# FintanH/rust-crdt

Hardware: AMD Instinct MI355X
Metric: replica-merges/sec (whole node) + achieved HBM GB/s as % of MI355X peak (higher is better)
Workload: dtype u64

## Files before the change

rust-crdt_amd/csrc/common.hpp:

```cpp
#pragma once

#include <hip/hip_runtime.h>

#include <cstdint>
#include <cstdio>
#include <algorithm>
#include <cstring>
#include <map>
#include <string>
#include <vector>

#include "crdt_gpu.h"
#include "shard_host.hpp"

namespace crdt {

using u64 = unsigned long long;
using u64x2 = unsigned long long __attribute__((ext_vector_type(2)));

constexpr int kWave = 64;

#ifndef CRDT_APPLY_WPE
#define CRDT_APPLY_WPE 0
#endif
// ... 62 lines not shown
  int wire_walk = 1;
  int wire_fill = 1;
  int host_stream = 1;
  int apply_lane = 1;
  int apply_fence = 0;
  int orswot_apply_pf = 0;
  int orswot_apply_stg = 0;
  int orswot_apply_l2pf = 0;
  int orswot_apply_meta = 1;
  int orswot_apply_hpf = 0;
  int map_counter_dma = 0;
  int map_counter_depth = 8;
  int map_counter_kpw = 0;
  int map_counter_cs = 1;
  int map_counter_cl = 0;
  int map_orswot_cs = 0;
  int map_orswot_wide = 0;
  int map_nested_lds = 1;
  int map_apply_meta = 1;
  int map_apply_pf = 1;
  int read_bpc = 0;
  int read_unroll = 8;
  int read_nt = 1;
  int eqv_ppl = 8;
  int eqv_bpc = 32;
  int rx_lds = 1;
};

struct PendingTiming {
  std::string name;
  hipEvent_t start, stop;
};

}

struct crdt_ctx {
  int device = 0;
  hipStream_t stream = nullptr;
  int cu_count = 256;
  bool timing = false;
  crdt::Tune tune;
  std::string last_error;
  void *scratch = nullptr;
  size_t scratch_bytes = 0;
  void *dscratch = nullptr;
  size_t dscratch_bytes = 0;
  unsigned *counters = nullptr;
  size_t counters_n = 0;
  void *pinned = nullptr;
  size_t pinned_bytes = 0;
  hipEvent_t pinned_done = nullptr;
  std::map<std::string, crdt::KernelTimer> timers;
  std::vector<crdt::PendingTiming> pending;
  std::vector<hipEvent_t> free_events;
  void *comm = nullptr;
  int nranks = 1, rank = 0;
  void (*comm_destroy)(void *) = nullptr;
  void *sbuf[8] = {};
  size_t sbuf_bytes[8] = {};
  bool has_ops = false;
  crdt_comm_ops ops{};
  hipStream_t astream = nullptr;
  hipEvent_t a_main = nullptr, a_done = nullptr;
  void *a_dev = nullptr, *a_host = nullptr;
  size_t a_rows = 0;
  std::string comm_note;
  void (*comm_release)(crdt_ctx *) = nullptr;
  crdt::shard_host::PlanCache plans;
  bool chk_pending = false;
  uint64_t chk_key = 0;
  void *chk_dev = nullptr;
  uint64_t *chk_host = nullptr;
  hipEvent_t chk_ev = nullptr;
  int (*comm_check)(crdt_ctx *) = nullptr;
  int mem_kind = CRDT_MEM_DEVICE;
  hipStream_t hstream = nullptr;
  void *hbuf[2] = {};
  size_t hbuf_bytes = 0;
  void *hacc = nullptr;
  size_t hacc_bytes = 0;
  hipEvent_t hcopied[2] = {}, hfree[2] = {};
};

namespace crdt {

int fail(crdt_ctx *ctx, int code, const char *fmt, ...);
int hip_fail(crdt_ctx *ctx, hipError_t e, const char *what);
int ensure_scratch(crdt_ctx *ctx, size_t bytes);
int ensure_dscratch(crdt_ctx *ctx, size_t bytes);
int ensure_counters(crdt_ctx *ctx, size_t n);
int stage_h2d(crdt_ctx *ctx, void *dst, const void *src, size_t bytes);
int device_fill(crdt_ctx *ctx, void *dst, size_t bytes, unsigned char byte);
void timing_begin(crdt_ctx *ctx, const char *name);
void timing_end(crdt_ctx *ctx);
void timing_add_host(crdt_ctx *ctx, const char *name, double ms);

struct DefPlan {
  const size_t *def_off;
  unsigned long long G, D, M, A, Mw;
  const u64 *def_clock, *def_members;
  const u64 *out_clock;
  u64 *out_entries;
  int apply_ceiling;
  u64 *hash;
  unsigned *surv;
  unsigned *nsurv;
  uint8_t *out_keep;
  u64 *out_members;
  u64 *tkey;
  unsigned *trep;
  unsigned long long tmask;
};
int launch_deferred(crdt_ctx *ctx, const size_t *host_def_off, DefPlan q, const u64 *dev_def_off = nullptr,
                    unsigned *status = nullptr);
int stage_def_off_dev(crdt_ctx *ctx, const u64 *src, size_t *dst, size_t G, size_t D, unsigned *status,
                      unsigned *flags);

enum class Op : int { Max = 0, Or = 1 };

template <Op OP>
__device__ __forceinline__ u64 join(u64 a, u64 b) {
  if constexpr (OP == Op::Max) return a > b ? a : b;
  else return a | b;
}
template <Op OP>
__device__ __forceinline__ u64x2 join2(u64x2 a, u64x2 b) {
  u64x2 r;
  r.x = join<OP>(a.x, b.x);
  r.y = join<OP>(a.y, b.y);
  return r;
}

int lattice_lub_many(crdt_ctx *ctx, Op op, const u64 *in, size_t G, size_t R, size_t W,
                     size_t row_stride, size_t group_stride, u64 *out, size_t out_stride,
                     unsigned flags);
int lattice_merge_batch(crdt_ctx *ctx, Op op, u64 *self, const u64 *other, size_t N, size_t W,
                        size_t self_stride, size_t other_stride);
struct LubReq {
  Op op;
  const u64 *in;
  size_t G, R, W, row_stride, group_stride;
  u64 *out;
  size_t out_stride;
  unsigned flags;
};
// ... 79 lines not shown
```

rust-crdt_amd/csrc/ctx.cpp:

```cpp
#include <cstdarg>
#include <cstdlib>

#include "common.hpp"

namespace crdt {

static thread_local std::string g_orphan_error;

int fail(crdt_ctx *ctx, int code, const char *fmt, ...) {
  char buf[512];
  va_list ap;
  va_start(ap, fmt);
  vsnprintf(buf, sizeof buf, fmt, ap);
  va_end(ap);
  if (ctx) ctx->last_error = buf;
  else g_orphan_error = buf;
  return code;
}

int hip_fail(crdt_ctx *ctx, hipError_t e, const char *what) {
  return fail(ctx, CRDT_EHIP, "%s failed: %s (%d)", what, hipGetErrorString(e), (int)e);
}

int ensure_scratch(crdt_ctx *ctx, size_t bytes) {
  if (bytes <= ctx->scratch_bytes) return CRDT_OK;
  if (ctx->scratch) {
    (void)hipStreamSynchronize(ctx->stream);
    (void)hipFree(ctx->scratch);
    ctx->scratch = nullptr;
    ctx->scratch_bytes = 0;
  }
  size_t want = bytes < (1u << 20) ? (1u << 20) : bytes + bytes / 4;
// ... 12 lines not shown
    (void)hipStreamSynchronize(ctx->stream);
    (void)hipFree(ctx->dscratch);
    ctx->dscratch = nullptr;
    ctx->dscratch_bytes = 0;
  }
  size_t want = bytes < (1u << 16) ? (1u << 16) : bytes + bytes / 4;
  hipError_t e = hipMalloc(&ctx->dscratch, want);
  if (e != hipSuccess) {
    ctx->dscratch = nullptr;
    return fail(ctx, CRDT_ENOMEM, "dscratch hipMalloc(%zu) failed: %s", want, hipGetErrorString(e));
  }
  ctx->dscratch_bytes = want;
  return CRDT_OK;
}

int ensure_counters(crdt_ctx *ctx, size_t n) {
  if (n <= ctx->counters_n) return CRDT_OK;
  if (ctx->counters) {
    (void)hipStreamSynchronize(ctx->stream);
    (void)hipFree(ctx->counters);
    ctx->counters = nullptr;
    ctx->counters_n = 0;
  }
  size_t want = n < 16384 ? 16384 : n * 2;
  hipError_t e = hipMalloc(&ctx->counters, want * sizeof(unsigned));
  if (e != hipSuccess) {
    ctx->counters = nullptr;
    return fail(ctx, CRDT_ENOMEM, "counter hipMalloc failed: %s", hipGetErrorString(e));
  }
  ctx->counters_n = want;
  return device_fill(ctx, ctx->counters, want * sizeof(unsigned), 0);
}

int stage_h2d(crdt_ctx *ctx, void *dst, const void *src, size_t bytes) {
  if (bytes == 0) return CRDT_OK;
  if (ctx->pinned_done) {
    hipError_t e = hipEventSynchronize(ctx->pinned_done);
    if (e != hipSuccess) return hip_fail(ctx, e, "hipEventSynchronize(pinned)");
  } else {
    hipError_t e = hipEventCreateWithFlags(&ctx->pinned_done, hipEventDisableTiming);
    if (e != hipSuccess) return hip_fail(ctx, e, "hipEventCreate(pinned)");
  }
  if (bytes > ctx->pinned_bytes) {
    if (ctx->pinned) (void)hipHostFree(ctx->pinned);
    ctx->pinned = nullptr;
    ctx->pinned_bytes = 0;
    size_t want = bytes < 65536 ? 65536 : bytes * 2;
    hipError_t e = hipHostMalloc(&ctx->pinned, want, hipHostMallocDefault);
    if (e != hipSuccess) return fail(ctx, CRDT_ENOMEM, "hipHostMalloc(%zu) failed", want);
    ctx->pinned_bytes = want;
  }
  std::memcpy(ctx->pinned, src, bytes);
  hipError_t e = hipMemcpyAsync(dst, ctx->pinned, bytes, hipMemcpyHostToDevice, ctx->stream);
  if (e != hipSuccess) return hip_fail(ctx, e, "hipMemcpyAsync(staged)");
  e = hipEventRecord(ctx->pinned_done, ctx->stream);
  if (e != hipSuccess) return hip_fail(ctx, e, "hipEventRecord(pinned)");
  return CRDT_OK;
}

__global__ void fill_u64_kernel(unsigned long long *p, size_t n, unsigned long long v) {
  for (size_t i = (size_t)blockIdx.x * blockDim.x + threadIdx.x; i < n; i += (size_t)gridDim.x * blockDim.x)
    p[i] = v;
}
__global__ void fill_u8_kernel(unsigned char *p, size_t n, unsigned char v) {
  for (size_t i = (size_t)blockIdx.x * blockDim.x + threadIdx.x; i < n; i += (size_t)gridDim.x * blockDim.x)
    p[i] = v;
}

int device_fill(crdt_ctx *ctx, void *dst, size_t bytes, unsigned char byte) {
  if (bytes == 0) return CRDT_OK;
  const bool wide = (reinterpret_cast<uintptr_t>(dst) % 8 == 0) && bytes % 8 == 0;
  const size_t n = wide ? bytes / 8 : bytes;
  size_t blocks = (n + kBlock - 1) / kBlock;
  const size_t cap = (size_t)ctx->cu_count * 8;
  if (blocks > cap) blocks = cap;
  if (wide)
    hipLaunchKernelGGL(fill_u64_kernel, dim3((unsigned)blocks), dim3(kBlock), 0, ctx->stream,
                       (unsigned long long *)dst, n, 0x0101010101010101ULL * byte);
  else
    hipLaunchKernelGGL(fill_u8_kernel, dim3((unsigned)blocks), dim3(kBlock), 0, ctx->stream,
                       (unsigned char *)dst, n, byte);
  hipError_t e = hipGetLastError();
  return e == hipSuccess ? CRDT_OK : hip_fail(ctx, e, "device_fill");
}

static hipEvent_t take_event(crdt_ctx *ctx) {
  if (!ctx->free_events.empty()) {
    hipEvent_t e = ctx->free_events.back();
    ctx->free_events.pop_back();
    return e;
// ... 135 lines not shown
int crdt_ctx_create(int device, crdt_ctx **out) {
  if (!out) return fail(nullptr, CRDT_EINVAL, "crdt_ctx_create: out is NULL");
  *out = nullptr;
  int n = 0;
  hipError_t e = hipGetDeviceCount(&n);
  if (e != hipSuccess || n == 0)
    return fail(nullptr, CRDT_EHIP, "crdt_ctx_create: no HIP device (%s)", hipGetErrorString(e));
  if (device < 0 || device >= n)
    return fail(nullptr, CRDT_EINVAL, "crdt_ctx_create: device %d out of range [0,%d)", device, n);
  e = hipSetDevice(device);
  if (e != hipSuccess) return hip_fail(nullptr, e, "hipSetDevice");
  auto *ctx = new crdt_ctx();
  ctx->device = device;
  hipDeviceProp_t prop;
  if (hipGetDeviceProperties(&prop, device) == hipSuccess && prop.multiProcessorCount > 0)
    ctx->cu_count = prop.multiProcessorCount;
  if (const char *t = getenv("CRDT_TUNE")) apply_tune(ctx, t);
  *out = ctx;
  return CRDT_OK;
}

int crdt_ctx_destroy(crdt_ctx *ctx) {
  if (!ctx) return CRDT_OK;
  (void)hipSetDevice(ctx->device);
  (void)hipStreamSynchronize(ctx->stream);
  for (auto &p : ctx->pending) {
    (void)hipEventDestroy(p.start);
    (void)hipEventDestroy(p.stop);
  }
  for (auto e : ctx->free_events) (void)hipEventDestroy(e);
  if (ctx->scratch) (void)hipFree(ctx->scratch);
  if (ctx->counters) (void)hipFree(ctx->counters);
  if (ctx->dscratch) (void)hipFree(ctx->dscratch);
  if (ctx->pinned) (void)hipHostFree(ctx->pinned);
  if (ctx->pinned_done) (void)hipEventDestroy(ctx->pinned_done);
  free_stage(ctx);
  if (ctx->comm && ctx->comm_destroy) ctx->comm_destroy(ctx->comm);
  if (ctx->comm_release) ctx->comm_release(ctx);
  for (void *b : ctx->sbuf)
    if (b) (void)hipFree(b);
  delete ctx;
  return CRDT_OK;
}

int crdt_ctx_set_stream(crdt_ctx *ctx, void *hip_stream) {
  CRDT_CHECK_CTX(ctx);
  ctx->stream = reinterpret_cast<hipStream_t>(hip_stream);
  return CRDT_OK;
}

int crdt_ctx_synchronize(crdt_ctx *ctx) {
  CRDT_CHECK_CTX(ctx);
  CRDT_HIP(ctx, hipSetDevice(ctx->device));
  CRDT_HIP(ctx, hipStreamSynchronize(ctx->stream));
  if (ctx->comm_check) return ctx->comm_check(ctx);
  return CRDT_OK;
}

const char *crdt_last_error(const crdt_ctx *ctx) {
  return ctx ? ctx->last_error.c_str() : g_orphan_error.c_str();
}

const char *crdt_version(void) { return "0.8.0"; }
int crdt_abi_version(void) { return CRDT_ABI_VERSION; }
const char *crdt_build_target(void) { return "gfx950"; }

int crdt_ctx_set_timing(crdt_ctx *ctx, int enable) {
  CRDT_CHECK_CTX(ctx);
// ... 30 lines not shown
```

rust-crdt_amd/csrc/map.hip:

```cpp
#include <type_traits>

#include "common.hpp"

namespace crdt {

struct MapPlan {
  const u64 *clock;
  long long c_rs, c_gs;
  const u64 *ec;
  long long e_rs, e_gs;
  const u64 *vclk;
  long long vc_rs, vc_gs;
  const u64 *vval;
  long long vv_rs, vv_gs;
  const size_t *def_off;
  const unsigned *def_row;
  const u64 *def_clock;
  const u64 *def_keys;
  unsigned long long G, R, K, A, V, Kw, Vout;
  u64 *o_clock, *o_ec, *o_vclk, *o_vval;
  unsigned *o_nval;
  unsigned *o_flags;
  int spec;
  int nt;
// ... 2181 lines not shown
  MapPlan p{};
  p.clock = (const u64 *)in->clock;
  p.c_rs = in->clock_rstride;
  p.c_gs = in->clock_gstride;
  p.ec = (const u64 *)in->ec;
  p.e_rs = in->ec_rstride;
  p.e_gs = in->ec_gstride;
  p.vclk = (const u64 *)in->vclk;
  p.vc_rs = in->vclk_rstride;
  p.vc_gs = in->vclk_gstride;
  p.vval = (const u64 *)in->vval;
  p.vv_rs = in->vval_rstride;
  p.vv_gs = in->vval_gstride;
  p.G = G;
  p.R = R;
  p.K = K;
  p.A = A;
  p.V = V;
  p.Kw = Kw;
  p.Vout = Vout;
  p.o_clock = (u64 *)out->clock;
  p.o_ec = (u64 *)out->ec;
  p.o_vclk = (u64 *)out->vclk;
  p.o_vval = (u64 *)out->vval;
  p.o_nval = out->nval;
  p.o_flags = out->flags;
  p.spec = ctx->tune.map_spec;
  p.nt = ctx->tune.map_nt;
  p.scan2 = ctx->tune.map_scan2 && A % 2 == 0;
  p.scan3 = ctx->tune.map_scan3;
  p.lazyv = ctx->tune.map_lazyv;
  p.batch = ctx->tune.map_batch;
  p.diag = ctx->tune.map_diag;
  if (int rc = device_fill(ctx, out->flags, G * sizeof(unsigned), 0)) return rc;
  const bool even = ((p.c_rs | p.c_gs | p.e_rs | p.e_gs | p.vc_rs | p.vc_gs) & 1) == 0;
  const bool glds = !wide && ctx->tune.map_glds && R > 0 && A <= 64 && (A & 1) == 0 && (V == 1 || V == 2) &&
                    want <= 4 && even && aligned16(p.clock) && aligned16(p.ec) && aligned16(p.vclk) &&
                    G * ((R + 7) / 8) < 0x7fffffffULL;
  const bool rs = glds && ctx->tune.map_rs && A <= 32;
  const unsigned gC = (!rs && ctx->tune.map_chunk == 8 && ctx->tune.map_ring == 4) ? 8 : 16;
  const size_t off_b = D > 0 || doff ? ((G + 1) * sizeof(size_t) + 255) / 256 * 256 : 0;
  if (glds) p.nch = (R + gC - 1) / gC;
  p.st = rs && ctx->tune.map_st && A == 32 && V == 2 && !(ctx->tune.map_sh && K % 4 == 0);
  const size_t cm_b = glds ? G * p.nch * A * sizeof(u64) : 0;
  const size_t cm_pad = (cm_b + 15) / 16 * 16, nv_b = deep && !out->nval ? G * K * sizeof(unsigned) : 0;
  if (off_b + cm_pad + nv_b > 0)
    if (int rc = ensure_scratch(ctx, off_b + cm_pad + nv_b)) return rc;
  crdt_map_out dout = *out;
  if (deep) {
    if (!dout.nval) dout.nval = reinterpret_cast<uint32_t *>(static_cast<char *>(ctx->scratch) + off_b + cm_pad);
    p.o_nval = map_deep_tag(dout.nval);
  }
  if (doff && D == 0)
    if (int rc = stage_def_off_dev(ctx, doff, (size_t *)ctx->scratch, G, 0, nullptr, out->flags)) return rc;
  if (D > 0) {
    if (doff) {
      if (int rc = stage_def_off_dev(ctx, doff, (size_t *)ctx->scratch, G, D, nullptr, out->flags)) return rc;
    } else if (int rc = stage_h2d(ctx, ctx->scratch, in->def_off, (G + 1) * sizeof(size_t))) {
      return rc;
    }
    p.def_off = reinterpret_cast<const size_t *>(ctx->scratch);
    p.def_row = in->def_row;
    p.def_clock = (const u64 *)in->def_clock;
    p.def_keys = (const u64 *)in->def_keys;
  }
  const unsigned long long blocks = G * K;
  hipError_t he;
  if (wide) {
    if (int rc = map_lub_wide(ctx, in, p.def_off, &dout, deep)) return rc;
    he = hipSuccess;
  } else {
  if (glds) {
    u64 *cm = reinterpret_cast<u64 *>(static_cast<char *>(ctx->scratch) + off_b);
    p.cmax = cm;
    timing_begin(ctx, "map_chunk_max");
    hipLaunchKernelGGL(map_chunk_max_kernel, dim3((unsigned)(G * p.nch)), dim3(64), 0, ctx->stream, p.clock,
                       p.c_rs, p.c_gs, (unsigned long long)R, (unsigned long long)A, p.nch, gC, cm);
    timing_end(ctx);
  }
  timing_begin(ctx, "map_fold");
  if (glds) {
    if (rs && ctx->tune.map_sh && A == 32 && V == 2 && K % 4 == 0)
      he = launch_map_sh(p, blocks, ctx->stream);
    else if (rs)
      he = V == 1 ? launch_map_rs<1>(p, blocks, ctx->stream) : launch_map_rs<2>(p, blocks, ctx->stream);
    else
      he = V == 1 ? launch_map_glds<1>(p, ctx->tune.map_chunk, ctx->tune.map_ring, blocks, ctx->stream)
                  : launch_map_glds<2>(p, ctx->tune.map_chunk, ctx->tune.map_ring, blocks, ctx->stream);
  } else {
    const int VI = map_vi(V, want);
    if (A <= 64) he = launch_map_vi<1>(p, VI, blocks, ctx->stream);
    else if (A <= 128) he = launch_map_vi<2>(p, VI, blocks, ctx->stream);
    else he = launch_map_vi<4>(p, VI, blocks, ctx->stream);
  }
  timing_end(ctx);
  }
  if (he != hipSuccess) return hip_fail(ctx, he, "map_fold_kernel launch");
  if (deep)
    if (int rc = map_lub_deep(ctx, in, p.def_off, &dout)) return rc;

  if (D == 0) return CRDT_OK;
  DefPlan q{};
  q.G = G;
  q.D = D;
  q.M = K;
  q.A = A;
  q.Mw = Kw;
  q.def_clock = (const u64 *)in->def_clock;
  q.def_members = (const u64 *)in->def_keys;
  q.out_clock = (const u64 *)out->clock;
  q.out_entries = nullptr;
  q.apply_ceiling = 0;
  q.out_keep = out->def_keep;
  q.out_members = (u64 *)out->def_keys;
  return launch_deferred(ctx, in->def_off, q, doff);
}

extern "C" int crdt_map_lub_many(crdt_ctx *ctx, const crdt_map_batch *in, crdt_map_out *out) {
  if (ctx && ctx->mem_kind == CRDT_MEM_HOST) return crdt::map_lub_many_host(ctx, in, out);
  CRDT_CHECK_CTX(ctx);
  if (!in || !out) return fail(ctx, CRDT_EINVAL, "map_lub_many: NULL batch/out");
  return map_lub_impl(ctx, in, nullptr, 0, out);
}

extern "C" int crdt_map_lub_many_doff(crdt_ctx *ctx, const crdt_map_batch *in, const uint64_t *def_off, size_t D,
                                      crdt_map_out *out) {
  CRDT_DEVICE_MEM_ONLY(ctx);
  CRDT_CHECK_CTX(ctx);
  if (!in || !out) return fail(ctx, CRDT_EINVAL, "map_lub_many_doff: NULL batch/out");
  if (in->def_off) return fail(ctx, CRDT_EINVAL, "map_lub_many_doff: in->def_off must be NULL");
  if (!def_off && D) return fail(ctx, CRDT_EINVAL, "map_lub_many_doff: D > 0 without def_off");
  return map_lub_impl(ctx, in, (const u64 *)def_off, D, out);
}
```

rust-crdt_amd/csrc/orswot.hip:

```cpp
#include "common.hpp"

namespace crdt {


template <int V>
struct OVec;
template <>
struct OVec<1> {
  using T = u64;
};
template <>
struct OVec<2> {
  using T = u64x2;
};

__device__ __forceinline__ u64 umax(u64 a, u64 b) { return a > b ? a : b; }

__device__ __forceinline__ u64 dot_join(u64 e1, u64 c1, u64 e2, u64 c2) {
  const u64 t0 = e1 == e2 ? e1 : 0;
  const u64 t1 = e1 > c2 ? e1 : 0;
  const u64 t2 = e2 > c1 ? e2 : 0;
  return umax(t0, umax(t1, t2));
}
__device__ __forceinline__ u64x2 dot_join(u64x2 e1, u64x2 c1, u64x2 e2, u64x2 c2) {
// ... 173 lines not shown
  if (s_flag & 2) {
    start(true);
    if (active) fold(0, p.R);
#if OR_VIOL_BALLOT
    viol |= vmask != 0;
#endif
  } else if (active) {
    c = VT(0);
#pragma unroll
    for (int j = 0; j < kOrMPT; ++j) e[j] = VT(0);
    const VT *pp = reinterpret_cast<const VT *>(p.part) + (size_t)u * p.S * slab;
    for (int k = 0; k < p.S; ++k, pp += slab) {
      const VT c2 = pp[(size_t)p.MB * kOrMPT * p.PW + cl];
#pragma unroll
      for (int j = 0; j < kOrMPT; ++j) e[j] = dot_join(e[j], c, pp[(ml + j * p.MB) * p.PW + cl], c2);
      c = umax(c, c2);
    }
  }
  store_final();
}


__device__ __forceinline__ unsigned long long group_of(const size_t *off, unsigned long long G,
                                                       unsigned long long d) {
  unsigned long long lo = 0, hi = G;
  while (hi - lo > 1) {
    const unsigned long long mid = (lo + hi) / 2;
    if (off[mid] <= d) lo = mid;
    else hi = mid;
  }
  return lo;
}

__global__ __launch_bounds__(kBlock) void orswot_deferred_kernel(DefPlan p) {
  __shared__ u64 s_hash[kBlock / kWave];
  const unsigned long long d = blockIdx.x;
  const unsigned long long g = group_of(p.def_off, p.G, d);
  const u64 *rm = p.def_clock + d * p.A;
  const u64 *cf = p.out_clock + g * p.A;
  int greater = 0;
  u64 h = 0;
  for (unsigned long long a = threadIdx.x; a < p.A; a += kBlock) {
    const u64 x = rm[a];
    greater |= x > cf[a];
    u64 z = x * 0x9E3779B97F4A7C15ULL + a;
    z = (z ^ (z >> 30)) * 0xBF58476D1CE4E5B9ULL;
    z = (z ^ (z >> 27)) * 0x94D049BB133111EBULL;
    h += z ^ (z >> 31);
  }
  const int keep = __syncthreads_or(greater);
  for (int off = kWave / 2; off > 0; off >>= 1) h += __shfl_down(h, off, kWave);
  if ((threadIdx.x & (kWave - 1)) == 0) s_hash[threadIdx.x / kWave] = h;
  const u64 *bits = p.def_members + d * p.Mw;
  u64 *E = p.out_entries + g * p.M * p.A;
  for (unsigned long long w = 0; w < p.Mw && p.apply_ceiling; ++w) {
    u64 word = bits[w];
    while (word) {
      const int bit = __builtin_ctzll(word);
      word &= word - 1;
      const unsigned long long m = w * 64 + bit;
      if (m >= p.M) break;
      u64 *row = E + m * p.A;
      for (unsigned long long a = threadIdx.x; a < p.A; a += kBlock) {
        const u64 e = row[a];
        if (e != 0 && e <= rm[a]) row[a] = 0;
      }
    }
  }
  __syncthreads();
  if (threadIdx.x == 0) {
    u64 t = 0;
    for (int w = 0; w < kBlock / kWave; ++w) t += s_hash[w];
    p.hash[d] = t;
    if (keep) p.surv[atomicAdd(p.nsurv, 1u)] = (unsigned)d;
  }
}

__device__ __forceinline__ u64 dedup_key(u64 h, unsigned long long g) {
  u64 z = h ^ ((g + 1) * 0x9E3779B97F4A7C15ULL);
  z = (z ^ (z >> 31)) * 0xD6E8FEB86659FD93ULL;
  z ^= z >> 32;
  return z ? z : 1;
}

__device__ __forceinline__ unsigned long long dedup_slot(const DefPlan &p, u64 key, bool insert, unsigned d) {
  unsigned long long t = key & p.tmask;
  while (true) {
    const u64 cur = insert ? atomicCAS(p.tkey + t, 0ull, key) : p.tkey[t];
    if (cur == key || (insert && cur == 0)) return t;
    if (!insert && cur == 0) return ~0ull;
    t = (t + 1) & p.tmask;
  }
}

__global__ __launch_bounds__(kBlock) void orswot_dedup_insert_kernel(DefPlan p) {
  const unsigned k = blockIdx.x * blockDim.x + threadIdx.x;
  const unsigned n = *p.nsurv;
  if (k >= n) return;
  const unsigned d = p.surv[k];
  const u64 key = dedup_key(p.hash[d], group_of(p.def_off, p.G, d));
  atomicMin(p.trep + dedup_slot(p, key, true, d), d);
}

__global__ __launch_bounds__(kBlock) void orswot_dedup_kernel(DefPlan p) {
  const unsigned k = blockIdx.x * blockDim.x + threadIdx.x;
  const unsigned n = *p.nsurv;
  if (k >= n) return;
  const unsigned d = p.surv[k];
  const unsigned long long g = group_of(p.def_off, p.G, d);
  const u64 key = dedup_key(p.hash[d], g);
  const unsigned long long t = dedup_slot(p, key, false, d);
  const u64 *rm = p.def_clock + (size_t)d * p.A;
  auto same = [&](unsigned d2) {
    if (d2 < p.def_off[g] || d2 >= p.def_off[g + 1]) return false;
    const u64 *rm2 = p.def_clock + (size_t)d2 * p.A;
    for (unsigned long long a = 0; a < p.A; ++a)
      if (rm[a] != rm2[a]) return false;
    return true;
  };
  unsigned rep = t == ~0ull ? d : p.trep[t];
  if (rep != d && !same(rep)) {
    rep = d;
    for (unsigned j = 0; j < n; ++j) {
      const unsigned d2 = p.surv[j];
      if (d2 < rep && p.hash[d2] == p.hash[d] && same(d2)) rep = d2;
    }
  }
  if (rep == d) p.out_keep[d] = 1;
  const u64 *src = p.def_members + (size_t)d * p.Mw;
  u64 *dst = p.out_members + (size_t)rep * p.Mw;
  for (unsigned long long w = 0; w < p.Mw; ++w)
    if (src[w]) atomicOr(dst + w, src[w]);
}

static bool al16(const void *p) { return (reinterpret_cast<uintptr_t>(p) & 15) == 0; }

__global__ __launch_bounds__(kBlock) void def_off_check_kernel(const u64 *src, size_t *dst, unsigned long long G,
                                                               unsigned long long D, unsigned *status,
                                                               unsigned *flags) {
  const unsigned long long i = (unsigned long long)blockIdx.x * kBlock + threadIdx.x;
  if (i > G) return;
  const u64 v = src[i];
  bool bad = i == 0 ? v != 0 : (i == G ? v != D : v > D);
  if (i > 0 && src[i - 1] > v) bad = true;
  dst[i] = i == 0 ? 0 : (i == G ? D : (v > D ? D : v));
  if (bad) {
    if (status) atomicOr(status, 1u);
    if (flags) {
      if (i > 0) atomicOr(flags + i - 1, 2u);
      if (i < G) atomicOr(flags + i, 2u);
    }
  }
}

int stage_def_off_dev(crdt_ctx *ctx, const u64 *src, size_t *dst, size_t G, size_t D, unsigned *status,
                      unsigned *flags) {
  const size_t n = G + 1;
  hipLaunchKernelGGL(def_off_check_kernel, dim3((unsigned)((n + kBlock - 1) / kBlock)), dim3(kBlock), 0,
                     ctx->stream, src, dst, (unsigned long long)G, (unsigned long long)D, status, flags);
  CRDT_HIP(ctx, hipGetLastError());
  return CRDT_OK;
}

int launch_deferred(crdt_ctx *ctx, const size_t *host_def_off, DefPlan q, const u64 *dev_def_off, unsigned *status) {
  const size_t G = q.G, D = q.D;
  const size_t off_b = (G + 1) * sizeof(size_t);
  size_t T = 64;
  while (T < 2 * D) T <<= 1;
  const size_t off_pad = (off_b + 255) / 256 * 256;
  const size_t need = 256 + off_pad + D * 8 + D * 4 + 64 + T * 12;
  if (int rc = ensure_dscratch(ctx, need)) return rc;
  char *base = static_cast<char *>(ctx->dscratch);
  q.nsurv = reinterpret_cast<unsigned *>(base);
  q.def_off = reinterpret_cast<const size_t *>(base + 256);
  q.hash = reinterpret_cast<u64 *>(base + 256 + off_pad);
  q.surv = reinterpret_cast<unsigned *>(q.hash + D);
  q.tkey = reinterpret_cast<u64 *>(base + ((256 + off_pad + D * 12 + 63) / 64 * 64));
  q.trep = reinterpret_cast<unsigned *>(q.tkey + T);
  q.tmask = T - 1;
  if (int rc = device_fill(ctx, q.tkey, T * 8, 0)) return rc;
  if (int rc = device_fill(ctx, q.trep, T * 4, 0xFF)) return rc;
  if (int rc = device_fill(ctx, q.nsurv, 4, 0)) return rc;
  if (dev_def_off) {
    if (int rc = stage_def_off_dev(ctx, dev_def_off, (size_t *)q.def_off, G, D, status, nullptr)) return rc;
  } else {
    int rc = stage_h2d(ctx, (void *)q.def_off, host_def_off, off_b);
    if (rc) return rc;
  }
  if (int rc = device_fill(ctx, q.out_keep, D, 0)) return rc;
  if (int rc = device_fill(ctx, q.out_members, D * q.Mw * 8, 0)) return rc;
  hipLaunchKernelGGL(orswot_deferred_kernel, dim3((unsigned)D), dim3(kBlock), 0, ctx->stream, q);
  hipLaunchKernelGGL(orswot_dedup_insert_kernel, dim3((unsigned)((D + kBlock - 1) / kBlock)), dim3(kBlock), 0,
                     ctx->stream, q);
  hipLaunchKernelGGL(orswot_dedup_kernel, dim3((unsigned)((D + kBlock - 1) / kBlock)), dim3(kBlock), 0,
                     ctx->stream, q);
  CRDT_HIP(ctx, hipGetLastError());
  return CRDT_OK;
}

}

using namespace crdt;

static int orswot_lub_impl(crdt_ctx *ctx, const crdt_orswot_batch *in, const u64 *doff, size_t Ddev,
                           crdt_orswot_out *out, unsigned *status, const OrswotJoinExtra *ex = nullptr) {
  const size_t G = in->G, R = in->R, M = in->M, A = in->A;
  if (G == 0 || A == 0) return CRDT_OK;
  if (!out->clock || (M && !out->entries)) return fail(ctx, CRDT_EINVAL, "orswot_lub_many: NULL output");
  if (R > 0 && (!in->clock || (M && !in->entries)))
    return fail(ctx, CRDT_EINVAL, "orswot_lub_many: NULL input");
  if (in->entry_mstride < A && M > 1)
    return fail(ctx, CRDT_EINVAL, "orswot_lub_many: entry_mstride < A");
  if (A > (1u << 20) || M > (1ull << 32))
    return fail(ctx, CRDT_EUNSUPPORTED, "orswot_lub_many: A or M too large");
  CRDT_HIP(ctx, hipSetDevice(ctx->device));
  const size_t D = doff ? Ddev : (in->def_off && G > 0) ? in->def_off[G] - in->def_off[0] : 0;
  if (in->def_off && in->def_off[0] != 0)
    return fail(ctx, CRDT_EINVAL, "orswot_lub_many: def_off[0] must be 0");
  const size_t Mw = (M + 63) / 64;
  if (D > 0 && (!in->def_clock || !out->def_keep || (Mw && (!in->def_members || !out->def_members))))
    return fail(ctx, CRDT_EINVAL, "orswot_lub_many: deferred buffers missing");
  if (D > 0xffffffffULL) return fail(ctx, CRDT_EUNSUPPORTED, "orswot_lub_many: too many deferred");

  if (ex && ex->viol)
    if (int rc = device_fill(ctx, ex->viol, G * 4, 0)) return rc;
  if (R == 0 && ex && ex->init_clock) {
    CRDT_HIP(ctx, hipMemcpyAsync(out->clock, ex->init_clock, G * A * 8, hipMemcpyDeviceToDevice, ctx->stream));
    if (M)
      CRDT_HIP(ctx, hipMemcpyAsync(out->entries, ex->init_entries, G * M * A * 8, hipMemcpyDeviceToDevice,
                                   ctx->stream));
  } else if (R == 0) {
    int rc = device_fill(ctx, out->clock, G * A * 8, 0);
    if (!rc && M) rc = device_fill(ctx, out->entries, G * M * A * 8, 0);
    if (rc) return rc;
  } else if (M == 0) {
    if (int rc = lattice_lub_many(ctx, Op::Max, (const u64 *)in->clock, G, R, A, in->clock_rstride,
                                  in->clock_gstride, (u64 *)out->clock, A, 0))
      return rc;
  } else {
    const bool vec2 = A % 2 == 0 && in->clock_rstride % 2 == 0 && in->clock_gstride % 2 == 0 &&
                      in->entry_mstride % 2 == 0 && in->entry_rstride % 2 == 0 &&
                      in->entry_gstride % 2 == 0 && al16(in->clock) && al16(in->entries) &&
                      al16(out->clock) && al16(out->entries) &&
                      (!ex || !ex->init_clock || (al16(ex->init_clock) && al16(ex->init_entries)));
    const int V = vec2 ? 2 : 1;
    OrPlan p{};
    p.clock = (const u64 *)in->clock;
    p.entries = (const u64 *)in->entries;
    p.c_rstride = in->clock_rstride;
    p.c_gstride = in->clock_gstride;
    p.e_mstride = in->entry_mstride;
    p.e_rstride = in->entry_rstride;
    p.e_gstride = in->entry_gstride;
    p.G = G;
    p.R = R;
    p.M = M;
    p.A = A;
    p.Wv = (int)(A / V);
// ... 28 lines not shown
    if (S > 1) {
      const size_t slab_b = (mpb * p.PW + p.PW) * V * 8;
      int rc = ensure_scratch(ctx, units * S * slab_b);
      if (rc) return rc;
      rc = ensure_counters(ctx, units);
      if (rc) return rc;
      p.cnt = ctx->counters;
      p.part = reinterpret_cast<u64 *>(ctx->scratch);
    }
    timing_begin(ctx, "orswot_join");
    const dim3 grid((unsigned)(units * S));
    const int UR = ctx->tune.orswot_unroll;
#define CRDT_ORJ(VV, UU, MM) hipLaunchKernelGGL((orswot_join_kernel<VV, UU, MM>), grid, dim3(kBlock), 0, ctx->stream, p)
    if (V == 2) {
      if (MPT == 4) {
        if (UR == 1) CRDT_ORJ(2, 1, 4);
        else if (UR == 4) CRDT_ORJ(2, 4, 4);
        else CRDT_ORJ(2, 2, 4);
      } else if (MPT == 8) {
        if (UR == 1) CRDT_ORJ(2, 1, 8);
        else CRDT_ORJ(2, 2, 8);
      } else {
        CRDT_ORJ(2, 1, 16);
      }
    } else {
      CRDT_ORJ(1, 2, 4);
    }
#undef CRDT_ORJ
    timing_end(ctx);
    CRDT_HIP(ctx, hipGetLastError());
  }

  if (D == 0) return CRDT_OK;
  DefPlan q{};
  q.G = G;
  q.D = D;
  q.M = M;
  q.A = A;
  q.Mw = Mw;
  q.def_clock = (const u64 *)in->def_clock;
  q.def_members = (const u64 *)in->def_members;
  q.out_clock = (const u64 *)out->clock;
  q.out_entries = (u64 *)out->entries;
  q.apply_ceiling = 1;
  q.out_keep = out->def_keep;
  q.out_members = (u64 *)out->def_members;
  return launch_deferred(ctx, in->def_off, q, doff, status);
}

namespace crdt {
int orswot_lub_many_ex(crdt_ctx *ctx, const crdt_orswot_batch *in, crdt_orswot_out *out, const OrswotJoinExtra &ex) {
  return orswot_lub_impl(ctx, in, nullptr, 0, out, nullptr, &ex);
}
}

extern "C" int crdt_orswot_lub_many(crdt_ctx *ctx, const crdt_orswot_batch *in,
                                    crdt_orswot_out *out) {
  if (ctx && ctx->mem_kind == CRDT_MEM_HOST) return crdt::orswot_lub_many_host(ctx, in, out);
  CRDT_CHECK_CTX(ctx);
  if (!in || !out) return fail(ctx, CRDT_EINVAL, "orswot_lub_many: NULL batch/out");
  return orswot_lub_impl(ctx, in, nullptr, 0, out, nullptr);
}

extern "C" int crdt_orswot_lub_many_doff(crdt_ctx *ctx, const crdt_orswot_batch *in, const uint64_t *def_off,
                                         size_t D, crdt_orswot_out *out, uint32_t *status) {
  CRDT_DEVICE_MEM_ONLY(ctx);
  CRDT_CHECK_CTX(ctx);
  if (!in || !out) return fail(ctx, CRDT_EINVAL, "orswot_lub_many_doff: NULL batch/out");
  if (in->def_off) return fail(ctx, CRDT_EINVAL, "orswot_lub_many_doff: in->def_off must be NULL");
  if (!def_off && D) return fail(ctx, CRDT_EINVAL, "orswot_lub_many_doff: D > 0 without def_off");
  CRDT_HIP(ctx, hipSetDevice(ctx->device));
  if (status)
    if (int rc = device_fill(ctx, status, sizeof(uint32_t), 0)) return rc;
  if (in->G == 0 || in->A == 0) return CRDT_OK;
  if (def_off && D == 0) {
    if (int rc = ensure_dscratch(ctx, (in->G + 1) * sizeof(size_t))) return rc;
    if (int rc = stage_def_off_dev(ctx, (const u64 *)def_off, (size_t *)ctx->dscratch, in->G, 0, status, nullptr))
      return rc;
    def_off = nullptr;
  }
// ... 3 lines not shown
```

Measured before the change: 2.283 billion.

## Fuse deferred-op prep fills, offset staging and chunk-max into one kernel

Replaces the several device_fill launches, the pinned H2D copy of def_off and the map chunk-max kernel with a single deferred_prepare kernel. That kernel zero-fills ranges, copies offsets straight from mapped pinned memory and computes chunk maxima. The pinned staging buffer becomes a ring of eight slots so the host no longer waits on the previous copy. The dedup insert kernel is folded into the deferred kernel, and the ceiling loop now spreads member rows across waves. The aim is to cut launch count and host sync overhead. The cost is zero-copy PCIe reads inside the kernel and more atomics in the deferred kernel.

Result: no change. 2.286 billion (median of 2 runs) (+0.1%).

```diff
diff --git a/rust-crdt_amd/csrc/common.hpp b/rust-crdt_amd/csrc/common.hpp
--- a/rust-crdt_amd/csrc/common.hpp
+++ b/rust-crdt_amd/csrc/common.hpp
@@ -118,6 +118,13 @@
   hipEvent_t start, stop;
 };
 
+struct StageSlot {
+  void *buf = nullptr;
+  size_t bytes = 0;
+  hipEvent_t done = nullptr;
+};
+constexpr int kStageSlots = 8;
+
 }
 
 struct crdt_ctx {
@@ -133,9 +140,8 @@
   size_t dscratch_bytes = 0;
   unsigned *counters = nullptr;
   size_t counters_n = 0;
-  void *pinned = nullptr;
-  size_t pinned_bytes = 0;
-  hipEvent_t pinned_done = nullptr;
+  crdt::StageSlot stage_slot[crdt::kStageSlots];
+  unsigned stage_next = 0;
   std::map<std::string, crdt::KernelTimer> timers;
   std::vector<crdt::PendingTiming> pending;
   std::vector<hipEvent_t> free_events;
@@ -176,6 +182,8 @@
 int ensure_dscratch(crdt_ctx *ctx, size_t bytes);
 int ensure_counters(crdt_ctx *ctx, size_t n);
 int stage_h2d(crdt_ctx *ctx, void *dst, const void *src, size_t bytes);
+int stage_pin(crdt_ctx *ctx, const void *src, size_t bytes, const void **dev_src, int *slot);
+int stage_pin_done(crdt_ctx *ctx, int slot);
 int device_fill(crdt_ctx *ctx, void *dst, size_t bytes, unsigned char byte);
 void timing_begin(crdt_ctx *ctx, const char *name);
 void timing_end(crdt_ctx *ctx);
@@ -197,6 +205,24 @@
   unsigned *trep;
   unsigned long long tmask;
 };
+struct FillRange {
+  void *p = nullptr;
+  size_t bytes = 0;
+  unsigned char byte = 0;
+};
+constexpr int kPrepExtra = 3;
+struct PrepExtra {
+  FillRange fill[kPrepExtra];
+  int nfill = 0;
+  const u64 *cm_clock = nullptr;
+  long long cm_rs = 0, cm_gs = 0;
+  unsigned long long cm_R = 0, cm_nch = 0;
+  unsigned cm_C = 0;
+  u64 *cm_out = nullptr;
+};
+int deferred_prepare(crdt_ctx *ctx, const size_t *host_def_off, DefPlan &q, const u64 *dev_def_off = nullptr,
+                     unsigned *status = nullptr, unsigned *flags = nullptr, const PrepExtra *extra = nullptr);
+int deferred_finish(crdt_ctx *ctx, const DefPlan &q);
 int launch_deferred(crdt_ctx *ctx, const size_t *host_def_off, DefPlan q, const u64 *dev_def_off = nullptr,
                     unsigned *status = nullptr);
 int stage_def_off_dev(crdt_ctx *ctx, const u64 *src, size_t *dst, size_t G, size_t D, unsigned *status,
diff --git a/rust-crdt_amd/csrc/ctx.cpp b/rust-crdt_amd/csrc/ctx.cpp
--- a/rust-crdt_amd/csrc/ctx.cpp
+++ b/rust-crdt_amd/csrc/ctx.cpp
@@ -1,3 +1,4 @@
+#include <chrono>
 #include <cstdarg>
 #include <cstdlib>
 
@@ -76,30 +77,64 @@
   return device_fill(ctx, ctx->counters, want * sizeof(unsigned), 0);
 }
 
+static int stage_take(crdt_ctx *ctx, const void *src, size_t bytes, int *slot) {
+  *slot = (int)ctx->stage_next;
+  StageSlot &s = ctx->stage_slot[ctx->stage_next];
+  ctx->stage_next = (ctx->stage_next + 1) % kStageSlots;
+  if (s.done) {
+    const auto t0 = std::chrono::steady_clock::now();
+    hipError_t e = hipEventSynchronize(s.done);
+    if (e != hipSuccess) return hip_fail(ctx, e, "hipEventSynchronize(stage slot)");
+    if (ctx->timing)
+      timing_add_host(ctx, "stage_wait",
+                      std::chrono::duration<double, std::milli>(std::chrono::steady_clock::now() - t0).count());
+  } else {
+    hipError_t e = hipEventCreateWithFlags(&s.done, hipEventDisableTiming);
+    if (e != hipSuccess) {
+      s.done = nullptr;
+      return hip_fail(ctx, e, "hipEventCreate(stage slot)");
+    }
+  }
+  if (bytes > s.bytes) {
+    if (s.buf) (void)hipHostFree(s.buf);
+    s.buf = nullptr;
+    s.bytes = 0;
+    size_t want = bytes < 65536 ? 65536 : bytes * 2;
+    hipError_t e = hipHostMalloc(&s.buf, want, hipHostMallocDefault);
+    if (e != hipSuccess) {
+      s.buf = nullptr;
+      return fail(ctx, CRDT_ENOMEM, "hipHostMalloc(%zu) failed", want);
+    }
+    s.bytes = want;
+  }
+  std::memcpy(s.buf, src, bytes);
+  return CRDT_OK;
+}
+
 int stage_h2d(crdt_ctx *ctx, void *dst, const void *src, size_t bytes) {
   if (bytes == 0) return CRDT_OK;
-  if (ctx->pinned_done) {
-    hipError_t e = hipEventSynchronize(ctx->pinned_done);
-    if (e != hipSuccess) return hip_fail(ctx, e, "hipEventSynchronize(pinned)");
-  } else {
-    hipError_t e = hipEventCreateWithFlags(&ctx->pinned_done, hipEventDisableTiming);
-    if (e != hipSuccess) return hip_fail(ctx, e, "hipEventCreate(pinned)");
-  }
-  if (bytes > ctx->pinned_bytes) {
-    if (ctx->pinned) (void)hipHostFree(ctx->pinned);
-    ctx->pinned = nullptr;
-    ctx->pinned_bytes = 0;
-    size_t want = bytes < 65536 ? 65536 : bytes * 2;
-    hipError_t e = hipHostMalloc(&ctx->pinned, want, hipHostMallocDefault);
-    if (e != hipSuccess) return fail(ctx, CRDT_ENOMEM, "hipHostMalloc(%zu) failed", want);
-    ctx->pinned_bytes = want;
-  }
-  std::memcpy(ctx->pinned, src, bytes);
-  hipError_t e = hipMemcpyAsync(dst, ctx->pinned, bytes, hipMemcpyHostToDevice, ctx->stream);
+  int slot = 0;
+  if (int rc = stage_take(ctx, src, bytes, &slot)) return rc;
+  StageSlot &s = ctx->stage_slot[slot];
+  hipError_t e = hipMemcpyAsync(dst, s.buf, bytes, hipMemcpyHostToDevice, ctx->stream);
   if (e != hipSuccess) return hip_fail(ctx, e, "hipMemcpyAsync(staged)");
-  e = hipEventRecord(ctx->pinned_done, ctx->stream);
-  if (e != hipSuccess) return hip_fail(ctx, e, "hipEventRecord(pinned)");
-  return CRDT_OK;
+  e = hipEventRecord(s.done, ctx->stream);
+  if (e != hipSuccess) return hip_fail(ctx, e, "hipEventRecord(stage slot)");
+  return CRDT_OK;
+}
+
+int stage_pin(crdt_ctx *ctx, const void *src, size_t bytes, const void **dev_src, int *slot) {
+  if (int rc = stage_take(ctx, src, bytes, slot)) return rc;
+  void *d = nullptr;
+  hipError_t e = hipHostGetDevicePointer(&d, ctx->stage_slot[*slot].buf, 0);
+  if (e != hipSuccess) return hip_fail(ctx, e, "hipHostGetDevicePointer(stage slot)");
+  *dev_src = d;
+  return CRDT_OK;
+}
+
+int stage_pin_done(crdt_ctx *ctx, int slot) {
+  hipError_t e = hipEventRecord(ctx->stage_slot[slot].done, ctx->stream);
+  return e == hipSuccess ? CRDT_OK : hip_fail(ctx, e, "hipEventRecord(stage slot)");
 }
 
 __global__ void fill_u64_kernel(unsigned long long *p, size_t n, unsigned long long v) {
@@ -301,8 +336,10 @@
   if (ctx->scratch) (void)hipFree(ctx->scratch);
   if (ctx->counters) (void)hipFree(ctx->counters);
   if (ctx->dscratch) (void)hipFree(ctx->dscratch);
-  if (ctx->pinned) (void)hipHostFree(ctx->pinned);
-  if (ctx->pinned_done) (void)hipEventDestroy(ctx->pinned_done);
+  for (auto &s : ctx->stage_slot) {
+    if (s.buf) (void)hipHostFree(s.buf);
+    if (s.done) (void)hipEventDestroy(s.done);
+  }
   free_stage(ctx);
   if (ctx->comm && ctx->comm_destroy) ctx->comm_destroy(ctx->comm);
   if (ctx->comm_release) ctx->comm_release(ctx);
diff --git a/rust-crdt_amd/csrc/map.hip b/rust-crdt_amd/csrc/map.hip
--- a/rust-crdt_amd/csrc/map.hip
+++ b/rust-crdt_amd/csrc/map.hip
@@ -2237,14 +2237,15 @@
   p.lazyv = ctx->tune.map_lazyv;
   p.batch = ctx->tune.map_batch;
   p.diag = ctx->tune.map_diag;
-  if (int rc = device_fill(ctx, out->flags, G * sizeof(unsigned), 0)) return rc;
+  if (D == 0)
+    if (int rc = device_fill(ctx, out->flags, G * sizeof(unsigned), 0)) return rc;
   const bool even = ((p.c_rs | p.c_gs | p.e_rs | p.e_gs | p.vc_rs | p.vc_gs) & 1) == 0;
   const bool glds = !wide && ctx->tune.map_glds && R > 0 && A <= 64 && (A & 1) == 0 && (V == 1 || V == 2) &&
                     want <= 4 && even && aligned16(p.clock) && aligned16(p.ec) && aligned16(p.vclk) &&
                     G * ((R + 7) / 8) < 0x7fffffffULL;
   const bool rs = glds && ctx->tune.map_rs && A <= 32;
   const unsigned gC = (!rs && ctx->tune.map_chunk == 8 && ctx->tune.map_ring == 4) ? 8 : 16;
-  const size_t off_b = D > 0 || doff ? ((G + 1) * sizeof(size_t) + 255) / 256 * 256 : 0;
+  const size_t off_b = D == 0 && doff ? ((G + 1) * sizeof(size_t) + 255) / 256 * 256 : 0;
   if (glds) p.nch = (R + gC - 1) / gC;
   p.st = rs && ctx->tune.map_st && A == 32 && V == 2 && !(ctx->tune.map_sh && K % 4 == 0);
   const size_t cm_b = glds ? G * p.nch * A * sizeof(u64) : 0;
@@ -2258,13 +2259,36 @@
   }
   if (doff && D == 0)
     if (int rc = stage_def_off_dev(ctx, doff, (size_t *)ctx->scratch, G, 0, nullptr, out->flags)) return rc;
+  u64 *cm = glds ? reinterpret_cast<u64 *>(static_cast<char *>(ctx->scratch) + off_b) : nullptr;
+  DefPlan q{};
   if (D > 0) {
-    if (doff) {
-      if (int rc = stage_def_off_dev(ctx, doff, (size_t *)ctx->scratch, G, D, nullptr, out->flags)) return rc;
-    } else if (int rc = stage_h2d(ctx, ctx->scratch, in->def_off, (G + 1) * sizeof(size_t))) {
-      return rc;
-    }
-    p.def_off = reinterpret_cast<const size_t *>(ctx->scratch);
+    q.G = G;
+    q.D = D;
+    q.M = K;
+    q.A = A;
+    q.Mw = Kw;
+    q.def_clock = (const u64 *)in->def_clock;
+    q.def_members = (const u64 *)in->def_keys;
+    q.out_clock = (const u64 *)out->clock;
+    q.out_entries = nullptr;
+    q.apply_ceiling = 0;
+    q.out_keep = out->def_keep;
+    q.out_members = (u64 *)out->def_keys;
+    PrepExtra px;
+    px.fill[0].p = out->flags;
+    px.fill[0].bytes = G * sizeof(unsigned);
+    px.nfill = 1;
+    if (glds) {
+      px.cm_clock = p.clock;
+      px.cm_rs = p.c_rs;
+      px.cm_gs = p.c_gs;
+      px.cm_R = R;
+      px.cm_nch = p.nch;
+      px.cm_C = gC;
+      px.cm_out = cm;
+    }
+    if (int rc = deferred_prepare(ctx, in->def_off, q, doff, nullptr, out->flags, &px)) return rc;
+    p.def_off = q.def_off;
     p.def_row = in->def_row;
     p.def_clock = (const u64 *)in->def_clock;
     p.def_keys = (const u64 *)in->def_keys;
@@ -2275,9 +2299,8 @@
     if (int rc = map_lub_wide(ctx, in, p.def_off, &dout, deep)) return rc;
     he = hipSuccess;
   } else {
-  if (glds) {
-    u64 *cm = reinterpret_cast<u64 *>(static_cast<char *>(ctx->scratch) + off_b);
-    p.cmax = cm;
+  if (glds) p.cmax = cm;
+  if (glds && D == 0) {
     timing_begin(ctx, "map_chunk_max");
     hipLaunchKernelGGL(map_chunk_max_kernel, dim3((unsigned)(G * p.nch)), dim3(64), 0, ctx->stream, p.clock,
                        p.c_rs, p.c_gs, (unsigned long long)R, (unsigned long long)A, p.nch, gC, cm);
@@ -2305,20 +2328,7 @@
     if (int rc = map_lub_deep(ctx, in, p.def_off, &dout)) return rc;
 
   if (D == 0) return CRDT_OK;
-  DefPlan q{};
-  q.G = G;
-  q.D = D;
-  q.M = K;
-  q.A = A;
-  q.Mw = Kw;
-  q.def_clock = (const u64 *)in->def_clock;
-  q.def_members = (const u64 *)in->def_keys;
-  q.out_clock = (const u64 *)out->clock;
-  q.out_entries = nullptr;
-  q.apply_ceiling = 0;
-  q.out_keep = out->def_keep;
-  q.out_members = (u64 *)out->def_keys;
-  return launch_deferred(ctx, in->def_off, q, doff);
+  return deferred_finish(ctx, q);
 }
 
 extern "C" int crdt_map_lub_many(crdt_ctx *ctx, const crdt_map_batch *in, crdt_map_out *out) {
diff --git a/rust-crdt_amd/csrc/orswot.hip b/rust-crdt_amd/csrc/orswot.hip
--- a/rust-crdt_amd/csrc/orswot.hip
+++ b/rust-crdt_amd/csrc/orswot.hip
@@ -229,6 +229,23 @@
   return lo;
 }
 
+__device__ __forceinline__ u64 dedup_key(u64 h, unsigned long long g) {
+  u64 z = h ^ ((g + 1) * 0x9E3779B97F4A7C15ULL);
+  z = (z ^ (z >> 31)) * 0xD6E8FEB86659FD93ULL;
+  z ^= z >> 32;
+  return z ? z : 1;
+}
+
+__device__ __forceinline__ unsigned long long dedup_slot(const DefPlan &p, u64 key, bool insert, unsigned d) {
+  unsigned long long t = key & p.tmask;
+  while (true) {
+    const u64 cur = insert ? atomicCAS(p.tkey + t, 0ull, key) : p.tkey[t];
+    if (cur == key || (insert && cur == 0)) return t;
+    if (!insert && cur == 0) return ~0ull;
+    t = (t + 1) & p.tmask;
+  }
+}
+
 __global__ __launch_bounds__(kBlock) void orswot_deferred_kernel(DefPlan p) {
   __shared__ u64 s_hash[kBlock / kWave];
   const unsigned long long d = blockIdx.x;
@@ -250,6 +267,8 @@
   if ((threadIdx.x & (kWave - 1)) == 0) s_hash[threadIdx.x / kWave] = h;
   const u64 *bits = p.def_members + d * p.Mw;
   u64 *E = p.out_entries + g * p.M * p.A;
+  const unsigned wave = threadIdx.x / kWave, lane = threadIdx.x % kWave;
+  unsigned nbit = 0;
   for (unsigned long long w = 0; w < p.Mw && p.apply_ceiling; ++w) {
     u64 word = bits[w];
     while (word) {
@@ -257,8 +276,9 @@
       word &= word - 1;
       const unsigned long long m = w * 64 + bit;
       if (m >= p.M) break;
+      if ((nbit++ & (kBlock / kWave - 1)) != wave) continue;
       u64 *row = E + m * p.A;
-      for (unsigned long long a = threadIdx.x; a < p.A; a += kBlock) {
+      for (unsigned long long a = lane; a < p.A; a += kWave) {
         const u64 e = row[a];
         if (e != 0 && e <= rm[a]) row[a] = 0;
       }
@@ -269,34 +289,11 @@
     u64 t = 0;
     for (int w = 0; w < kBlock / kWave; ++w) t += s_hash[w];
     p.hash[d] = t;
-    if (keep) p.surv[atomicAdd(p.nsurv, 1u)] = (unsigned)d;
-  }
-}
-
-__device__ __forceinline__ u64 dedup_key(u64 h, unsigned long long g) {
-  u64 z = h ^ ((g + 1) * 0x9E3779B97F4A7C15ULL);
-  z = (z ^ (z >> 31)) * 0xD6E8FEB86659FD93ULL;
-  z ^= z >> 32;
-  return z ? z : 1;
-}
-
-__device__ __forceinline__ unsigned long long dedup_slot(const DefPlan &p, u64 key, bool insert, unsigned d) {
-  unsigned long long t = key & p.tmask;
-  while (true) {
-    const u64 cur = insert ? atomicCAS(p.tkey + t, 0ull, key) : p.tkey[t];
-    if (cur == key || (insert && cur == 0)) return t;
-    if (!insert && cur == 0) return ~0ull;
-    t = (t + 1) & p.tmask;
-  }
-}
-
-__global__ __launch_bounds__(kBlock) void orswot_dedup_insert_kernel(DefPlan p) {
-  const unsigned k = blockIdx.x * blockDim.x + threadIdx.x;
-  const unsigned n = *p.nsurv;
-  if (k >= n) return;
-  const unsigned d = p.surv[k];
-  const u64 key = dedup_key(p.hash[d], group_of(p.def_off, p.G, d));
-  atomicMin(p.trep + dedup_slot(p, key, true, d), d);
+    if (keep) {
+      p.surv[atomicAdd(p.nsurv, 1u)] = (unsigned)d;
+      atomicMin(p.trep + dedup_slot(p, dedup_key(t, g), true, (unsigned)d), (unsigned)d);
+    }
+  }
 }
 
 __global__ __launch_bounds__(kBlock) void orswot_dedup_kernel(DefPlan p) {
@@ -359,7 +356,60 @@
   return CRDT_OK;
 }
 
-int launch_deferred(crdt_ctx *ctx, const size_t *host_def_off, DefPlan q, const u64 *dev_def_off, unsigned *status) {
+constexpr int kPrepFill = 5 + kPrepExtra;
+struct PrepPlan {
+  FillRange fill[kPrepFill];
+  int nfill;
+  unsigned zblocks;
+  const size_t *off_src;
+  size_t *off_dst;
+  unsigned long long off_n;
+  const u64 *cm_clock;
+  long long cm_rs, cm_gs;
+  unsigned long long cm_R, cm_A, cm_nch, cm_units;
+  unsigned cm_C;
+  u64 *cm_out;
+};
+
+__global__ __launch_bounds__(kBlock) void deferred_prepare_kernel(PrepPlan pp) {
+  if (blockIdx.x >= pp.zblocks) {
+    const unsigned long long u = (unsigned long long)(blockIdx.x - pp.zblocks) * (kBlock / kWave) + threadIdx.x / kWave;
+    if (u >= pp.cm_units) return;
+    const unsigned long long g = u / pp.cm_nch, ch = u % pp.cm_nch;
+    const unsigned long long i0 = ch * pp.cm_C, i1 = pp.cm_R < i0 + pp.cm_C ? pp.cm_R : i0 + pp.cm_C;
+    for (unsigned long long a = threadIdx.x % kWave; a < pp.cm_A; a += kWave) {
+      u64 m = 0;
+      for (unsigned long long i = i0; i < i1; ++i) {
+        const u64 x = __builtin_nontemporal_load(pp.cm_clock + g * pp.cm_gs + i * pp.cm_rs + a);
+        m = m > x ? m : x;
+      }
+      pp.cm_out[u * pp.cm_A + a] = m;
+    }
+    return;
+  }
+  const size_t tid = (size_t)blockIdx.x * kBlock + threadIdx.x, nth = (size_t)pp.zblocks * kBlock;
+  if (pp.off_src)
+    for (size_t i = tid; i < pp.off_n; i += nth) pp.off_dst[i] = pp.off_src[i];
+#pragma unroll
+  for (int r = 0; r < kPrepFill; ++r) {
+    if (r >= pp.nfill) break;
+    unsigned char *p = static_cast<unsigned char *>(pp.fill[r].p);
+    const size_t bytes = pp.fill[r].bytes;
+    const unsigned char v = pp.fill[r].byte;
+    size_t head = (16 - (reinterpret_cast<uintptr_t>(p) & 15)) & 15;
+    if (head > bytes) head = bytes;
+    const size_t body = (bytes - head) / 16;
+    for (size_t i = tid; i < head; i += nth) p[i] = v;
+    u64x2 vv;
+    vv.x = vv.y = 0x0101010101010101ULL * v;
+    u64x2 *q = reinterpret_cast<u64x2 *>(p + head);
+    for (size_t i = tid; i < body; i += nth) q[i] = vv;
+    for (size_t i = head + body * 16 + tid; i < bytes; i += nth) p[i] = v;
+  }
+}
+
+int deferred_prepare(crdt_ctx *ctx, const size_t *host_def_off, DefPlan &q, const u64 *dev_def_off, unsigned *status,
+                     unsigned *flags, const PrepExtra *extra) {
   const size_t G = q.G, D = q.D;
   const size_t off_b = (G + 1) * sizeof(size_t);
   size_t T = 64;
@@ -375,24 +425,72 @@
   q.tkey = reinterpret_cast<u64 *>(base + ((256 + off_pad + D * 12 + 63) / 64 * 64));
   q.trep = reinterpret_cast<unsigned *>(q.tkey + T);
   q.tmask = T - 1;
-  if (int rc = device_fill(ctx, q.tkey, T * 8, 0)) return rc;
-  if (int rc = device_fill(ctx, q.trep, T * 4, 0xFF)) return rc;
-  if (int rc = device_fill(ctx, q.nsurv, 4, 0)) return rc;
-  if (dev_def_off) {
-    if (int rc = stage_def_off_dev(ctx, dev_def_off, (size_t *)q.def_off, G, D, status, nullptr)) return rc;
-  } else {
-    int rc = stage_h2d(ctx, (void *)q.def_off, host_def_off, off_b);
-    if (rc) return rc;
-  }
-  if (int rc = device_fill(ctx, q.out_keep, D, 0)) return rc;
-  if (int rc = device_fill(ctx, q.out_members, D * q.Mw * 8, 0)) return rc;
+  PrepPlan pp{};
+  int slot = -1;
+  if (!dev_def_off) {
+    const void *src = nullptr;
+    if (int rc = stage_pin(ctx, host_def_off, off_b, &src, &slot)) return rc;
+    pp.off_src = static_cast<const size_t *>(src);
+    pp.off_dst = const_cast<size_t *>(q.def_off);
+    pp.off_n = G + 1;
+  }
+  auto add = [&](void *p, size_t bytes, unsigned char byte) {
+    if (!p || bytes == 0) return;
+    pp.fill[pp.nfill].p = p;
+    pp.fill[pp.nfill].bytes = bytes;
+    pp.fill[pp.nfill].byte = byte;
+    ++pp.nfill;
+  };
+  add(q.tkey, T * 8, 0);
+  add(q.trep, T * 4, 0xFF);
+  add(q.nsurv, 16, 0);
+  add(q.out_keep, D, 0);
+  add(q.out_members, D * q.Mw * 8, 0);
+  if (extra) {
+    if (extra->nfill < 0 || extra->nfill > kPrepExtra) return fail(ctx, CRDT_EINVAL, "deferred_prepare: %d extra ranges", extra->nfill);
+    for (int i = 0; i < extra->nfill; ++i) add(extra->fill[i].p, extra->fill[i].bytes, extra->fill[i].byte);
+  }
+  size_t pieces = 0;
+  for (int i = 0; i < pp.nfill; ++i) pieces += (pp.fill[i].bytes + 15) / 16;
+  size_t zblocks = (pieces + kBlock - 1) / kBlock;
+  const size_t cap = (size_t)ctx->cu_count * 8;
+  if (zblocks > cap) zblocks = cap;
+  pp.zblocks = (unsigned)zblocks;
+  size_t cblocks = 0;
+  if (extra && extra->cm_out) {
+    pp.cm_clock = extra->cm_clock;
+    pp.cm_rs = extra->cm_rs;
+    pp.cm_gs = extra->cm_gs;
+    pp.cm_R = extra->cm_R;
+    pp.cm_A = q.A;
+    pp.cm_nch = extra->cm_nch;
+    pp.cm_units = G * extra->cm_nch;
+    pp.cm_C = extra->cm_C;
+    pp.cm_out = extra->cm_out;
+    cblocks = (pp.cm_units + kBlock / kWave - 1) / (kBlock / kWave);
+  }
+  if (zblocks + cblocks > 0x7fffffffULL) return fail(ctx, CRDT_EUNSUPPORTED, "deferred_prepare: grid too large");
+  hipLaunchKernelGGL(deferred_prepare_kernel, dim3((unsigned)(zblocks + cblocks)), dim3(kBlock), 0, ctx->stream, pp);
+  CRDT_HIP(ctx, hipGetLastError());
+  if (slot >= 0)
+    if (int rc = stage_pin_done(ctx, slot)) return rc;
+  if (dev_def_off)
+    if (int rc = stage_def_off_dev(ctx, dev_def_off, (size_t *)q.def_off, G, D, status, flags)) return rc;
+  return CRDT_OK;
+}
+
+int deferred_finish(crdt_ctx *ctx, const DefPlan &q) {
+  const size_t D = q.D;
   hipLaunchKernelGGL(orswot_deferred_kernel, dim3((unsigned)D), dim3(kBlock), 0, ctx->stream, q);
-  hipLaunchKernelGGL(orswot_dedup_insert_kernel, dim3((unsigned)((D + kBlock - 1) / kBlock)), dim3(kBlock), 0,
-                     ctx->stream, q);
   hipLaunchKernelGGL(orswot_dedup_kernel, dim3((unsigned)((D + kBlock - 1) / kBlock)), dim3(kBlock), 0,
                      ctx->stream, q);
   CRDT_HIP(ctx, hipGetLastError());
   return CRDT_OK;
+}
+
+int launch_deferred(crdt_ctx *ctx, const size_t *host_def_off, DefPlan q, const u64 *dev_def_off, unsigned *status) {
+  if (int rc = deferred_prepare(ctx, host_def_off, q, dev_def_off, status)) return rc;
+  return deferred_finish(ctx, q);
 }
 
 }
@@ -419,8 +517,30 @@
     return fail(ctx, CRDT_EINVAL, "orswot_lub_many: deferred buffers missing");
   if (D > 0xffffffffULL) return fail(ctx, CRDT_EUNSUPPORTED, "orswot_lub_many: too many deferred");
 
-  if (ex && ex->viol)
+  DefPlan q{};
+  if (D > 0) {
+    q.G = G;
+    q.D = D;
+    q.M = M;
+    q.A = A;
+    q.Mw = Mw;
+    q.def_clock = (const u64 *)in->def_clock;
+    q.def_members = (const u64 *)in->def_members;
+    q.out_clock = (const u64 *)out->clock;
+    q.out_entries = (u64 *)out->entries;
+    q.apply_ceiling = 1;
+    q.out_keep = out->def_keep;
+    q.out_members = (u64 *)out->def_members;
+    PrepExtra px;
+    if (ex && ex->viol) {
+      px.fill[0].p = ex->viol;
+      px.fill[0].bytes = G * 4;
+      px.nfill = 1;
+    }
+    if (int rc = deferred_prepare(ctx, in->def_off, q, doff, status, nullptr, &px)) return rc;
+  } else if (ex && ex->viol) {
     if (int rc = device_fill(ctx, ex->viol, G * 4, 0)) return rc;
+  }
   if (R == 0 && ex && ex->init_clock) {
     CRDT_HIP(ctx, hipMemcpyAsync(out->clock, ex->init_clock, G * A * 8, hipMemcpyDeviceToDevice, ctx->stream));
     if (M)
@@ -515,20 +635,7 @@
   }
 
   if (D == 0) return CRDT_OK;
-  DefPlan q{};
-  q.G = G;
-  q.D = D;
-  q.M = M;
-  q.A = A;
-  q.Mw = Mw;
-  q.def_clock = (const u64 *)in->def_clock;
-  q.def_members = (const u64 *)in->def_members;
-  q.out_clock = (const u64 *)out->clock;
-  q.out_entries = (u64 *)out->entries;
-  q.apply_ceiling = 1;
-  q.out_keep = out->def_keep;
-  q.out_members = (u64 *)out->def_members;
-  return launch_deferred(ctx, in->def_off, q, doff, status);
+  return deferred_finish(ctx, q);
 }
 
 namespace crdt {
```
